# zouyunkai/MedicalSemSeg

Measured on AMD Instinct MI355X. Metric: 96^3 vols/sec fwd+bwd (train), higher is better.
Workload: dtype bf16; 1 GPU; UNet base (MONAI BasicUNet 32-32-64-128-256-32) 1->3cls, 96^3 patches, DiceCE + AdamW, per-GPU batch 2; global_batch=2, parallelism=dp1, grad_sync=none (single rank)

## Files before the change

medicalsemseg_amd/csrc/common.h:

```cpp
#pragma once
#include <hip/hip_runtime.h>
#include <stdint.h>
#include <stdio.h>

#include "../../include/msseg.h"

typedef __bf16 bf16_t;
typedef __attribute__((ext_vector_type(8))) __bf16 bf16x8_t;
typedef __attribute__((ext_vector_type(4))) __bf16 bf16x4_t;
typedef __attribute__((ext_vector_type(4))) float f32x4_t;
typedef __attribute__((ext_vector_type(4))) uint32_t u32x4_t;
typedef __attribute__((ext_vector_type(2))) uint32_t u32x2_t;

#define MSSEG_DEVFN __device__ __forceinline__

void msseg_set_error(const char* fmt, ...);
#define MSSEG_FAIL(code, ...)           \
    do {                                \
        msseg_set_error(__VA_ARGS__);   \
        return (code);                  \
    } while (0)
#define MSSEG_CHECK_LAUNCH(name)                                              \
    do {                                                                      \
        hipError_t e__ = hipGetLastError();                                   \
        if (e__ != hipSuccess) MSSEG_FAIL(MSSEG_ELAUNCH, "%s: %s", name, hipGetErrorString(e__)); \
    } while (0)

bool msseg_ktimer_on();
int msseg_ktimer_begin(const char* name, hipStream_t stream);
void msseg_ktimer_end(int slot, hipStream_t stream);
#define MSSEG_KTIMED(name, stream, launch_stmt)                               \
    do {                                                                      \
        const int kt__ = msseg_ktimer_on() ? msseg_ktimer_begin(name, stream) : -1; \
        launch_stmt;                                                          \
        if (kt__ >= 0) msseg_ktimer_end(kt__, stream);                        \
    } while (0)

#include <atomic>
struct msseg_lds_attr_once {
    std::atomic<unsigned long long> done{0};
    bool ensure(const void* kern, int bytes) {
        int dev = 0;
        if (hipGetDevice(&dev) != hipSuccess) return false;
        const bool tracked = dev >= 0 && dev < 64;
        if (tracked && ((done.load(std::memory_order_acquire) >> dev) & 1ull)) return true;
        if (hipFuncSetAttribute(kern, hipFuncAttributeMaxDynamicSharedMemorySize, bytes) != hipSuccess) return false;
        if (tracked) done.fetch_or(1ull << dev, std::memory_order_release);
        return true;
    }
};

template <typename T> struct DT;
template <> struct DT<float> {
    static constexpr int EPC = 4;
    static constexpr int CODE = MSSEG_F32;
    static MSSEG_DEVFN float ld(const float* p) { return *p; }
    static MSSEG_DEVFN void st(float* p, float v) { *p = v; }
};
template <> struct DT<bf16_t> {
    static constexpr int EPC = 8;
    static constexpr int CODE = MSSEG_BF16;
    static MSSEG_DEVFN float ld(const bf16_t* p) { return (float)*p; }
    static MSSEG_DEVFN void st(bf16_t* p, float v) { *p = (bf16_t)v; }
};

template <typename T> MSSEG_DEVFN void mma_chunk(f32x4_t& acc, const u32x4_t& a, const u32x4_t& b);
template <> MSSEG_DEVFN void mma_chunk<bf16_t>(f32x4_t& acc, const u32x4_t& a, const u32x4_t& b) {
    acc = __builtin_amdgcn_mfma_f32_16x16x32_bf16(__builtin_bit_cast(bf16x8_t, a), __builtin_bit_cast(bf16x8_t, b),
                                                  acc, 0, 0, 0);
}
template <> MSSEG_DEVFN void mma_chunk<float>(f32x4_t& acc, const u32x4_t& a, const u32x4_t& b) {
    f32x4_t af = __builtin_bit_cast(f32x4_t, a), bf = __builtin_bit_cast(f32x4_t, b);
#pragma unroll
    for (int j = 0; j < 4; ++j) acc = __builtin_amdgcn_mfma_f32_16x16x4f32(af[j], bf[j], acc, 0, 0, 0);
}

MSSEG_DEVFN u32x4_t ldg16(const void* p) { return *(const u32x4_t*)p; }

MSSEG_DEVFN long long wimg_frag_off(int blk, int nkb, int kb, int q, int cb, int row) {
    return ((((long long)blk * nkb + kb) * 4 + q) * cb + row) * 16;
}
MSSEG_DEVFN long long wimg_kblock_bytes(int cb) { return (long long)4 * cb * 16; }

MSSEG_DEVFN bf16x4_t lds_tr_read(const unsigned char* p) {
    return __builtin_amdgcn_ds_read_tr16_b64_v4bf16(
        (__attribute__((address_space(3))) bf16x4_t*)(uintptr_t)(uint32_t)(uintptr_t)p);
}
MSSEG_DEVFN u32x4_t tr_frag(const unsigned char* base, int r0, int r1) {
    const bf16x4_t lo = lds_tr_read(base + r0), hi = lds_tr_read(base + r1);
    const bf16x8_t f = {lo[0], lo[1], lo[2], lo[3], hi[0], hi[1], hi[2], hi[3]};
    return __builtin_bit_cast(u32x4_t, f);
}

static inline bool msseg_aligned_bf16(int dtype, const void* a, long long lda, int ca, const void* b, long long ldb, int cb) {
    return dtype == MSSEG_BF16 && !((lda % 8) || (ldb % 8) || ((uintptr_t)a & 15) || ((uintptr_t)b & 15) || lda < ca || ldb < cb);
}

template <typename T> struct Chunk;
template <> struct Chunk<bf16_t> {
    static constexpr int E = 8;
    static MSSEG_DEVFN void load(const bf16_t* p, float* f) {
        const bf16x8_t v = *(const bf16x8_t*)p;
#pragma unroll
        for (int e = 0; e < 8; ++e) f[e] = (float)v[e];
    }
    static MSSEG_DEVFN void store(bf16_t* p, const float* f) {
        bf16x8_t v;
#pragma unroll
        for (int e = 0; e < 8; ++e) v[e] = (bf16_t)f[e];
        *(bf16x8_t*)p = v;
    }
};
template <> struct Chunk<float> {
    static constexpr int E = 4;
    static MSSEG_DEVFN void load(const float* p, float* f) {
        const f32x4_t v = *(const f32x4_t*)p;
#pragma unroll
        for (int e = 0; e < 4; ++e) f[e] = v[e];
    }
    static MSSEG_DEVFN void store(float* p, const float* f) { *(f32x4_t*)p = f32x4_t{f[0], f[1], f[2], f[3]}; }
};

template <typename T> MSSEG_DEVFN void load4(const T* p, float* f);
template <> MSSEG_DEVFN void load4<float>(const float* p, float* f) { Chunk<float>::load(p, f); }
template <> MSSEG_DEVFN void load4<bf16_t>(const bf16_t* p, float* f) {
    const bf16x4_t v = *(const bf16x4_t*)p;
#pragma unroll
    for (int e = 0; e < 4; ++e) f[e] = (float)v[e];
}
template <typename T> MSSEG_DEVFN void store4(T* p, const float* f);
template <> MSSEG_DEVFN void store4<float>(float* p, const float* f) { Chunk<float>::store(p, f); }
template <> MSSEG_DEVFN void store4<bf16_t>(bf16_t* p, const float* f) {
    *(bf16x4_t*)p = bf16x4_t{(bf16_t)f[0], (bf16_t)f[1], (bf16_t)f[2], (bf16_t)f[3]};
}

MSSEG_DEVFN float wave_sum(float v) {
#pragma unroll
    for (int o = 32; o > 0; o >>= 1) v += __shfl_xor(v, o);
    return v;
}

MSSEG_DEVFN bool grid_last_block(unsigned int* counter, unsigned int total_blocks, int* lds_flag) {
    asm volatile("s_waitcnt vmcnt(0)" ::: "memory");
    __syncthreads();
    if (threadIdx.x == 0) {
        __builtin_amdgcn_fence(__ATOMIC_RELEASE, "agent");
        asm volatile("s_waitcnt vmcnt(0)" ::: "memory");
        const unsigned int prev = __hip_atomic_fetch_add(counter, 1u, __ATOMIC_RELAXED, __HIP_MEMORY_SCOPE_AGENT);
        const int last = (prev == total_blocks - 1u) ? 1 : 0;
        if (last) {
            __builtin_amdgcn_fence(__ATOMIC_ACQUIRE, "agent");
            asm volatile("s_waitcnt vmcnt(0)" ::: "memory");
            __hip_atomic_store(counter, 0u, __ATOMIC_RELAXED, __HIP_MEMORY_SCOPE_AGENT);
        }
        *lds_flag = last;
    }
    __syncthreads();
    return *lds_flag != 0;
}

template <int NT>
MSSEG_DEVFN void block_rows_sum(const float* rows, int R, int L, float* lds, long long stride = 0) {
    const int tid = threadIdx.x, q = L >> 2;
    const int SL = NT / q;
    const int c4 = tid % q, slot = tid / q;
    const long long q_stride = (stride ? stride : (long long)L) >> 2;
    f32x4_t* l4 = (f32x4_t*)lds;
    if (slot < SL) {
        f32x4_t acc = {0.f, 0.f, 0.f, 0.f};
        const f32x4_t* src = (const f32x4_t*)rows + c4;
#pragma unroll 8
        for (int x = slot; x < R; x += SL) acc += src[(long long)x * q_stride];
        l4[slot * q + c4] = acc;
    }
    __syncthreads();
    if (tid < q) {
        f32x4_t t = {0.f, 0.f, 0.f, 0.f};
        for (int sl = 0; sl < SL; ++sl) t += l4[sl * q + tid];
        l4[NT + tid] = t;
    }
    __syncthreads();
}

#define MSSEG_SCRATCH_COUNTER_BYTES 256
#define MSSEG_STATS_NMAX 8

static inline int scratch_ok(const void* scratch, size_t bytes, const char* who) {
    if (!scratch || ((uintptr_t)scratch & 255) || bytes < msseg_reduce_scratch_bytes())
        MSSEG_FAIL(MSSEG_EWORKSPACE, "%s: needs a zero-initialised, 256-byte aligned scratch of %zu bytes", who,
                   msseg_reduce_scratch_bytes());
    return MSSEG_OK;
}

static inline int ceil_div(int a, int b) { return (a + b - 1) / b; }
static inline long long ceil_div_ll(long long a, long long b) { return (a + b - 1) / b; }

static inline int stream_grid(long long items, long long items_per_block = 256) {
    long long b = ceil_div_ll(items, items_per_block);
    const long long cap = (long long)msseg_num_cus() * 16;
    if (b > cap) b = cap;
    return (int)(b < 1 ? 1 : b);
}

static inline int epc_of(int dtype) { return dtype == MSSEG_F32 ? 4 : 8; }

template <typename T> struct type_tag { using type = T; };
template <typename F> static inline bool for_dtype(int dtype, F&& f) {
    if (dtype == MSSEG_F32) f(type_tag<float>{});
    else if (dtype == MSSEG_BF16) f(type_tag<bf16_t>{});
    else return false;
    return true;
}
```

medicalsemseg_amd/csrc/elementwise.hip:

```cpp
#include "common.h"

#include <stdarg.h>
#include <string.h>

static thread_local char g_err[512] = "";
void msseg_set_error(const char* fmt, ...) {
    va_list ap;
    va_start(ap, fmt);
    vsnprintf(g_err, sizeof(g_err), fmt, ap);
    va_end(ap);
}

extern "C" {
int msseg_abi_version(void) { return MSSEG_ABI_VERSION; }
const char* msseg_last_error(void) { return g_err; }
int msseg_num_cus(void) {
    static int cus = 0;
    if (cus == 0) {
        int dev = 0;
        hipDeviceProp_t prop;
        if (hipGetDevice(&dev) == hipSuccess && hipGetDeviceProperties(&prop, dev) == hipSuccess)
            cus = prop.multiProcessorCount;
        if (cus <= 0) cus = 256;
    }
    return cus;
}
}

namespace {

template <typename T> struct ChunkV {
    static constexpr int EPC = DT<T>::EPC;
    float v[EPC];
    MSSEG_DEVFN void load(const T* p) { Chunk<T>::load(p, v); }
    MSSEG_DEVFN void store(T* p) const { Chunk<T>::store(p, v); }
};

inline bool vec_ok(const void* p, long long ld, int C, int esz) {
    const int epc = 16 / esz;
    return (C % epc) == 0 && (ld % epc) == 0 && (((uintptr_t)p) & 15) == 0;
}

struct RowMap {
    int groups;
    int rows_par;
};
inline RowMap row_map(int C, int width, int nthr = 256) {
    RowMap m;
    m.groups = ceil_div(C, width);
    if (m.groups > nthr) m.groups = nthr;
    m.rows_par = nthr / m.groups;
    if (m.rows_par < 1) m.rows_par = 1;
    return m;
}

MSSEG_DEVFN void finalize_channels(const float* ws, int N, int nblk, int C, int nper, int mode, float* out,
                                   float* dp0, float* dp1, int accumulate) {
    __shared__ float fin[256];
    const int L = C * nper;
    const int cols = L < 256 ? L : 256;
    const int G = 256 / cols;
    const int col = threadIdx.x % cols, rg = threadIdx.x / cols;
    const bool in256 = threadIdx.x < 256;
    const int n_step = mode == 0 ? (int)gridDim.y : 1, n_first = mode == 0 ? (int)blockIdx.y : 0;
    for (int c0 = blockIdx.x * cols; c0 < L; c0 += gridDim.x * cols) {
        const int o = c0 + col;
        const bool ok = in256 && o < L && rg < G;
        float tot = 0.f;
        for (int n = n_first; n < N; n += n_step) {
            float s = 0.f;
            if (ok) {
                const float* src = ws + (long long)n * nblk * L + o;
#pragma unroll 16
                for (int bb = rg; bb < nblk; bb += G) s += src[(long long)bb * L];
            }
            __syncthreads();
            if (in256) fin[threadIdx.x] = s;
            __syncthreads();
            if (ok && rg == 0) {
                float t = 0.f;
                for (int g = 0; g < G; ++g) t += fin[g * cols + col];
                if (mode != 1) out[(long long)n * L + o] = t;
                tot += t;
            }
        }
        if (ok && rg == 0) {
            if (mode == 1) {
                out[o] = accumulate ? out[o] + tot : tot;
            } else if (mode == 2) {
                const int c = o / nper, k = o % nper;
                float* dp = (k == 0) ? dp0 : dp1;
                if (dp) dp[c] = accumulate ? dp[c] + tot : tot;
            }
        }
    }
}

struct FinalizeArgs {
    const float* ws; int N, nblk, C, nper, mode; float* out; float* dp0; float* dp1; int accumulate;
};
__global__ __launch_bounds__(256) void channels_finalize_kernel(const FinalizeArgs a) {
    finalize_channels(a.ws, a.N, a.nblk, a.C, a.nper, a.mode, a.out, a.dp0, a.dp1, a.accumulate);
}

static inline dim3 channels_finalize_grid(const FinalizeArgs& a) {
    const int L = a.C * a.nper;
    int gx = (L + 255) / 256;
    if (gx > 64) gx = 64;
    if (gx < 1) gx = 1;
    return dim3((unsigned)gx, a.mode == 0 ? (unsigned)(a.N < 1 ? 1 : a.N) : 1u);
}

constexpr int RED_THREADS = 512;
constexpr int RED_STAGE2 = 16;

template <int W>
MSSEG_DEVFN void block_rows_reduce(float* red, int groups, int rows_par, int g, int rl, bool act) {
    if (act && rl < RED_STAGE2 && rl < rows_par) {
#pragma unroll
        for (int e = 0; e < W; ++e) {
            float a = 0.f, b = 0.f;
            for (int k = rl; k < rows_par; k += RED_STAGE2) {
                a += red[((k * groups + g) * W + e) * 2 + 0];
                b += red[((k * groups + g) * W + e) * 2 + 1];
            }
            red[((rl * groups + g) * W + e) * 2 + 0] = a;
            red[((rl * groups + g) * W + e) * 2 + 1] = b;
        }
    }
    __syncthreads();
}

template <typename T, bool VEC>
__global__ __launch_bounds__(RED_THREADS) void channel_stats_kernel(const T* __restrict__ x, long long ldx, float* out,
                                                            long long S, int C, int groups, int rows_par,
                                                            long long rows_per_block, int nacc, int accumulate,
                                                            float* ws, unsigned int* counter) {
    constexpr int W = VEC ? DT<T>::EPC : 1;
    __shared__ float red[RED_THREADS * 2 * (VEC ? DT<T>::EPC : 1)];
    __shared__ int lflag;
    const int n = blockIdx.y;
    const int g = threadIdx.x % groups, rl = threadIdx.x / groups;
    const long long r0 = (long long)blockIdx.x * rows_per_block;
    long long r1 = r0 + rows_per_block;
    if (r1 > S) r1 = S;
    const T* xn = x + (long long)n * S * ldx;
    float* wsb = ws + ((long long)n * gridDim.x + blockIdx.x) * C * nacc;
    for (int gbase = 0; gbase * W < C; gbase += groups) {
        const int gg = gbase + g;
        const bool act = gg * W < C;
        float s[W], s2[W];
#pragma unroll
        for (int e = 0; e < W; ++e) s[e] = s2[e] = 0.f;
        if (act && rl < rows_par) {
#pragma unroll 8
            for (long long r = r0 + rl; r < r1; r += rows_par) {
// ... 179 lines not shown
    var = var > 0.f ? var : 0.f;
    rstd = rsqrtf(var + eps);
}

template <typename T, bool VEC, int MODE>
__global__ __launch_bounds__(MODE == 1 ? RED_THREADS : 256) void instnorm_kernel(const NormParams p) {
    constexpr int W = VEC ? DT<T>::EPC : 1;
    __shared__ float red[(MODE == 1) ? RED_THREADS * 2 * W : 1];
    __shared__ int lflag;
    const int n = blockIdx.y;
    const int g = threadIdx.x % p.groups, rl = threadIdx.x / p.groups;
    const long long r0 = (long long)blockIdx.x * p.rows_per_block;
    long long r1 = r0 + p.rows_per_block;
    if (r1 > p.S) r1 = p.S;
    const T* xn = (const T*)p.x + (long long)n * p.S * p.ldx;
    const T* yn = (MODE != 0 && p.y != nullptr) ? (const T*)p.y + (long long)n * p.S * p.ldy : nullptr;
    T* yo = (MODE == 0) ? (T*)p.y + (long long)n * p.S * p.ldy : nullptr;
    const T* dyn = (MODE != 0) ? (const T*)p.dy + (long long)n * p.S * p.lddy : nullptr;
    const T* resn = (MODE == 0 && p.res) ? (const T*)p.res + (long long)n * p.S * p.ldr : nullptr;
    T* dxn = (MODE == 2) ? (T*)p.dx + (long long)n * p.S * p.lddx : nullptr;
    T* drn = (MODE == 2 && p.dres) ? (T*)p.dres + (long long)n * p.S * p.lddres : nullptr;
    const float invS = 1.0f / (float)p.S;

    for (int gbase = 0; gbase * W < p.C; gbase += p.groups) {
        const int gg = gbase + g;
        const bool act = gg * W < p.C;
        float mean[W], rstd[W], sc[W], sh[W], k0[W], k1[W], a0[W], a1[W];
#pragma unroll
        for (int e = 0; e < W; ++e) {
            const int c = act ? gg * W + e : 0;
            mean_rstd(p.stats, n, p.C, c, p.S, p.eps, mean[e], rstd[e]);
            const float ga = p.gamma ? p.gamma[c] : 1.f;
            sc[e] = rstd[e] * ga;
            sh[e] = (p.beta ? p.beta[c] : 0.f) - mean[e] * sc[e];
            a0[e] = a1[e] = 0.f;
            if constexpr (MODE == 2) {
                k0[e] = p.red[((long long)n * p.C + c) * 2 + 0] * invS;
                k1[e] = p.red[((long long)n * p.C + c) * 2 + 1] * invS;
            }
        }
        if (act && rl < p.rows_par) {
#pragma unroll 4
            for (long long r = r0 + rl; r < r1; r += p.rows_par) {
                float xv[W], o[W], yv[W], dv[W];
                if constexpr (VEC) {
                    ChunkV<T> c; c.load(xn + r * p.ldx + gg * W);
#pragma unroll
                    for (int e = 0; e < W; ++e) xv[e] = c.v[e];
                } else {
                    xv[0] = DT<T>::ld(xn + r * p.ldx + gg);
                }
                if constexpr (MODE == 0) {
                    float rv[W];
#pragma unroll
                    for (int e = 0; e < W; ++e) rv[e] = 0.f;
                    if (resn) {
                        if constexpr (VEC) {
                            ChunkV<T> c; c.load(resn + r * p.ldr + gg * W);
#pragma unroll
                            for (int e = 0; e < W; ++e) rv[e] = c.v[e];
                        } else {
                            rv[0] = DT<T>::ld(resn + r * p.ldr + gg);
                        }
                    }
#pragma unroll
                    for (int e = 0; e < W; ++e) {
                        const float z = xv[e] * sc[e] + sh[e] + rv[e];
                        o[e] = z > 0.f ? z : z * p.slope;
                    }
                    if constexpr (VEC) {
                        ChunkV<T> c;
#pragma unroll
                        for (int e = 0; e < W; ++e) c.v[e] = o[e];
                        c.store(yo + r * p.ldy + gg * W);
                    } else {
                        DT<T>::st(yo + r * p.ldy + gg, o[0]);
                    }
                } else {
                    if constexpr (VEC) {
                        ChunkV<T> d; d.load(dyn + r * p.lddy + gg * W);
#pragma unroll
                        for (int e = 0; e < W; ++e) dv[e] = d.v[e];
                        if (yn != nullptr) {
                            ChunkV<T> c; c.load(yn + r * p.ldy + gg * W);
#pragma unroll
                            for (int e = 0; e < W; ++e) yv[e] = c.v[e];
                        } else {
#pragma unroll
                            for (int e = 0; e < W; ++e) yv[e] = xv[e] * sc[e] + sh[e];
                        }
                    } else {
                        dv[0] = DT<T>::ld(dyn + r * p.lddy + gg);
                        yv[0] = (yn != nullptr) ? DT<T>::ld(yn + r * p.ldy + gg) : xv[0] * sc[0] + sh[0];
                    }
#pragma unroll
                    for (int e = 0; e < W; ++e) {
                        const float dz = yv[e] > 0.f ? dv[e] : dv[e] * p.slope;
                        const float xh = (xv[e] - mean[e]) * rstd[e];
                        if constexpr (MODE == 1) {
                            a0[e] += dz;
                            a1[e] += dz * xh;
                        } else {
                            o[e] = sc[e] * (dz - k0[e] - xh * k1[e]);
                            dv[e] = dz;
                        }
                    }
                    if constexpr (MODE == 2) {
                        if constexpr (VEC) {
                            ChunkV<T> c;
#pragma unroll
                            for (int e = 0; e < W; ++e) c.v[e] = o[e];
                            c.store(dxn + r * p.lddx + gg * W);
                            if (drn) {
#pragma unroll
                                for (int e = 0; e < W; ++e) c.v[e] = dv[e];
                                c.store(drn + r * p.lddres + gg * W);
                            }
                        } else {
                            DT<T>::st(dxn + r * p.lddx + gg, o[0]);
                            if (drn) DT<T>::st(drn + r * p.lddres + gg, dv[0]);
                        }
                    }
                }
            }
        }
        if constexpr (MODE == 1) {
            __syncthreads();
#pragma unroll
            for (int e = 0; e < W; ++e) {
                red[(threadIdx.x * W + e) * 2 + 0] = a0[e];
                red[(threadIdx.x * W + e) * 2 + 1] = a1[e];
            }
            __syncthreads();
            block_rows_reduce<W>(red, p.groups, p.rows_par, g, rl, act);
            if (act && rl == 0) {
                const int kmax = p.rows_par < RED_STAGE2 ? p.rows_par : RED_STAGE2;
#pragma unroll
                for (int e = 0; e < W; ++e) {
                    float a = 0.f, b = 0.f;
                    for (int k = 0; k < kmax; ++k) {
                        a += red[((k * p.groups + g) * W + e) * 2 + 0];
                        b += red[((k * p.groups + g) * W + e) * 2 + 1];
                    }
                    const int c = gg * W + e;
                    float* wsb = p.ws + ((long long)n * gridDim.x + blockIdx.x) * p.C * 2;
                    wsb[c * 2 + 0] = a;
                    wsb[c * 2 + 1] = b;
                }
            }
        }
    }
}

struct NormPoolParams {
    const void* x; long long ldx;
    const float* stats; const float* gamma; const float* beta;
    void* y; long long ldy;
    void* pooled; long long ldp;
    int N, D, H, W, C; float eps, slope;
};

template <typename T>
__global__ __launch_bounds__(256) void instnorm_pool_fwd_kernel(const NormPoolParams p) {
    constexpr int WD = DT<T>::EPC;
    const int OD = p.D / 2, OH = p.H / 2, OW = p.W / 2;
    const unsigned ug = (unsigned)(p.C / WD);
    const unsigned total = (unsigned)((long long)p.N * OD * OH * OW * ug);
    const long long S = (long long)p.D * p.H * p.W;
    for (unsigned i = blockIdx.x * 256u + threadIdx.x; i < total; i += gridDim.x * 256u) {
        unsigned t = i / ug;
        const int g = (int)(i - t * ug);
        unsigned t2 = t / (unsigned)OW;
        const int ow = (int)(t - t2 * (unsigned)OW);
        t = t2 / (unsigned)OH;
        const int oh = (int)(t2 - t * (unsigned)OH);
        const int n = (int)(t / (unsigned)OD);
        const int od = (int)(t - (unsigned)n * (unsigned)OD);
        float sc[WD], sh[WD], best[WD];
#pragma unroll
        for (int e = 0; e < WD; ++e) {
            const int c = g * WD + e;
            float mean, rstd;
            mean_rstd(p.stats, n, p.C, c, S, p.eps, mean, rstd);
            sc[e] = rstd * (p.gamma ? p.gamma[c] : 1.f);
            sh[e] = (p.beta ? p.beta[c] : 0.f) - mean * sc[e];
            best[e] = -INFINITY;
        }
        ChunkV<T> in[8];
#pragma unroll
        for (int k = 0; k < 8; ++k) {
            const long long vox = (((long long)n * p.D + 2 * od + (k >> 2)) * p.H + 2 * oh + ((k >> 1) & 1)) * p.W + 2 * ow + (k & 1);
            in[k].load((const T*)p.x + vox * p.ldx + g * WD);
        }
#pragma unroll
        for (int k = 0; k < 8; ++k) {
            const long long vox = (((long long)n * p.D + 2 * od + (k >> 2)) * p.H + 2 * oh + ((k >> 1) & 1)) * p.W + 2 * ow + (k & 1);
            ChunkV<T> o;
#pragma unroll
            for (int e = 0; e < WD; ++e) {
                const float z = in[k].v[e] * sc[e] + sh[e];
                const float a = (float)(T)(z > 0.f ? z : z * p.slope);
                o.v[e] = a;
                if (a > best[e] || a != a) best[e] = a;
            }
            o.store((T*)p.y + vox * p.ldy + g * WD);
        }
        ChunkV<T> b;
#pragma unroll
        for (int e = 0; e < WD; ++e) b.v[e] = best[e];
        const long long ovox = (((long long)n * OD + od) * OH + oh) * OW + ow;
        b.store((T*)p.pooled + ovox * p.ldp + g * WD);
    }
}

struct NormPoolBwdParams {
    const void* x; long long ldx;
    const float* stats; const float* gamma; const float* beta;
    const void* skip; long long lds;
    const void* g; long long ldg;
    void* da; long long ldda;
    int N, D, H, W, C; float eps, slope;
    int groups, rows_par; long long cells_per_block;
    float* ws;
};

template <typename T>
__global__ __launch_bounds__(RED_THREADS) void instnorm_poolbwd_reduce_kernel(const NormPoolBwdParams p) {
    constexpr int WD = DT<T>::EPC;
    __shared__ float red[RED_THREADS * 2 * WD];
    const int n = blockIdx.y;
    const int g = threadIdx.x % p.groups, rl = threadIdx.x / p.groups;
    const int OD = p.D / 2, OH = p.H / 2, OW = p.W / 2;
    const long long cells = (long long)OD * OH * OW, S = (long long)p.D * p.H * p.W;
    const long long c0 = (long long)blockIdx.x * p.cells_per_block;
    long long c1 = c0 + p.cells_per_block;
    if (c1 > cells) c1 = cells;
    const T* xn = (const T*)p.x + (long long)n * S * p.ldx;
    const T* sn = (const T*)p.skip + (long long)n * S * p.lds;
    const T* gn = (const T*)p.g + (long long)n * cells * p.ldg;
    T* dn = (T*)p.da + (long long)n * S * p.ldda;
    for (int gbase = 0; gbase * WD < p.C; gbase += p.groups) {
        const int gg = gbase + g;
        const bool act = gg * WD < p.C;
        float mean[WD], rstd[WD], sc[WD], sh[WD], a0[WD], a1[WD];
#pragma unroll
        for (int e = 0; e < WD; ++e) {
            const int c = act ? gg * WD + e : 0;
            mean_rstd(p.stats, n, p.C, c, S, p.eps, mean[e], rstd[e]);
            sc[e] = rstd[e] * (p.gamma ? p.gamma[c] : 1.f);
            sh[e] = (p.beta ? p.beta[c] : 0.f) - mean[e] * sc[e];
            a0[e] = a1[e] = 0.f;
        }
        if (act && rl < p.rows_par) {
            for (long long cell = c0 + rl; cell < c1; cell += p.rows_par) {
                const int ow = (int)(cell % OW), oh = (int)((cell / OW) % OH), od = (int)(cell / ((long long)OW * OH));
                ChunkV<T> xin[8], gv;
                ChunkV<T> skin[8];
                long long vox[8];
#pragma unroll
                for (int k = 0; k < 8; ++k) {
                    vox[k] = ((long long)(2 * od + (k >> 2)) * p.H + 2 * oh + ((k >> 1) & 1)) * p.W + 2 * ow + (k & 1);
                    xin[k].load(xn + vox[k] * p.ldx + gg * WD);
                }
#pragma unroll
                for (int k = 0; k < 8; ++k) skin[k].load(sn + vox[k] * p.lds + gg * WD);
                gv.load(gn + cell * p.ldg + gg * WD);
                float best[WD];
                int arg[WD];
#pragma unroll
                for (int e = 0; e < WD; ++e) { best[e] = -INFINITY; arg[e] = 0; }
#pragma unroll
                for (int k = 0; k < 8; ++k) {
#pragma unroll
                    for (int e = 0; e < WD; ++e) {
                        const float z = xin[k].v[e] * sc[e] + sh[e];
                        const float a = (float)(T)(z > 0.f ? z : z * p.slope);
                        if (a > best[e] || a != a) { best[e] = a; arg[e] = k; }
                    }
                }
#pragma unroll
                for (int k = 0; k < 8; ++k) {
                    ChunkV<T> o;
#pragma unroll
                    for (int e = 0; e < WD; ++e) {
                        const float dv = (float)(T)(skin[k].v[e] + (arg[e] == k ? gv.v[e] : 0.f));
                        o.v[e] = dv;
                        const float z = xin[k].v[e] * sc[e] + sh[e];
                        const float dz = z > 0.f ? dv : dv * p.slope;
                        a0[e] += dz;
                        a1[e] += dz * ((xin[k].v[e] - mean[e]) * rstd[e]);
                    }
                    o.store(dn + vox[k] * p.ldda + gg * WD);
                }
            }
        }
        __syncthreads();
#pragma unroll
        for (int e = 0; e < WD; ++e) {
            red[(threadIdx.x * WD + e) * 2 + 0] = a0[e];
            red[(threadIdx.x * WD + e) * 2 + 1] = a1[e];
        }
        __syncthreads();
        block_rows_reduce<WD>(red, p.groups, p.rows_par, g, rl, act);
        if (act && rl == 0) {
            const int kmax = p.rows_par < RED_STAGE2 ? p.rows_par : RED_STAGE2;
#pragma unroll
            for (int e = 0; e < WD; ++e) {
                float a = 0.f, b = 0.f;
                for (int k = 0; k < kmax; ++k) {
                    a += red[((k * p.groups + g) * WD + e) * 2 + 0];
                    b += red[((k * p.groups + g) * WD + e) * 2 + 1];
                }
                float* wsb = p.ws + ((long long)n * gridDim.x + blockIdx.x) * p.C * 2;
                wsb[(gg * WD + e) * 2 + 0] = a;
                wsb[(gg * WD + e) * 2 + 1] = b;
            }
        }
    }
}

struct HeadBwdParams {
    const void* dy; long long lddy;
    const float* w;
    const void* x; long long ldx;
    const float* stats; const float* gamma; const float* beta;
    void* da; long long ldda;
    long long S; int C, Cout; float eps, slope;
    int groups, rows_par; long long rows_per_block;
    float* ws;
    int want_dw;
};

struct HeadFinArgs {
    const float* ws; int N, nblk, C, nper, Cout; float* red; float* dbeta; float* dgamma; float* dw; int acc_norm, acc_dw;
};
__global__ __launch_bounds__(256) void head_finalize_kernel(const HeadFinArgs a) {
    __shared__ __attribute__((aligned(16))) float fin[256 * 4 + 64 * 6];
    __shared__ float tot_n[64 * 6];
    const int L = a.C * a.nper;
    for (int o = threadIdx.x; o < L; o += 256) tot_n[o] = 0.f;
    for (int n = 0; n < a.N; ++n) {
        block_rows_sum<256>(a.ws + (long long)n * a.nblk * L, a.nblk, L, fin);
        const float* t = fin + 256 * 4;
        for (int o = threadIdx.x; o < L; o += 256) {
            const int c = o / a.nper, k = o % a.nper;
            if (k < 2) a.red[((long long)n * a.C + c) * 2 + k] = t[o];
            tot_n[o] += t[o];
        }
        __syncthreads();
    }
    for (int o = threadIdx.x; o < L; o += 256) {
        const int c = o / a.nper, k = o % a.nper;
        const float tot = tot_n[o];
        if (k == 0) { if (a.dbeta) a.dbeta[c] = a.acc_norm ? a.dbeta[c] + tot : tot; }
        else if (k == 1) { if (a.dgamma) a.dgamma[c] = a.acc_norm ? a.dgamma[c] + tot : tot; }
        else if (k - 2 < a.Cout && a.dw) a.dw[(k - 2) * a.C + c] = a.acc_dw ? a.dw[(k - 2) * a.C + c] + tot : tot;
    }
}

template <typename T, bool DW>
__global__ __launch_bounds__(RED_THREADS) void head_dgrad_inbwd_kernel(const HeadBwdParams p) {
    constexpr int WD = DT<T>::EPC;
    __shared__ float red[RED_THREADS * 2 * WD];
    const int n = blockIdx.y;
    const int g = threadIdx.x % p.groups, rl = threadIdx.x / p.groups;
    const long long r0 = (long long)blockIdx.x * p.rows_per_block;
    long long r1 = r0 + p.rows_per_block;
    if (r1 > p.S) r1 = p.S;
    const T* xn = (const T*)p.x + (long long)n * p.S * p.ldx;
    const T* dyn = (const T*)p.dy + (long long)n * p.S * p.lddy;
    T* dan = (T*)p.da + (long long)n * p.S * p.ldda;
    for (int gbase = 0; gbase * WD < p.C; gbase += p.groups) {
        const int gg = gbase + g;
        const bool act = gg * WD < p.C;
        float mean[WD], rstd[WD], sc[WD], sh[WD], a0[WD], a1[WD], wv[4][WD];
        float gw[DW ? 4 : 1][WD];
#pragma unroll
        for (int e = 0; e < WD; ++e) {
            const int c = act ? gg * WD + e : 0;
            mean_rstd(p.stats, n, p.C, c, p.S, p.eps, mean[e], rstd[e]);
            sc[e] = rstd[e] * (p.gamma ? p.gamma[c] : 1.f);
            sh[e] = (p.beta ? p.beta[c] : 0.f) - mean[e] * sc[e];
            a0[e] = a1[e] = 0.f;
#pragma unroll
            for (int k = 0; k < 4; ++k) wv[k][e] = k < p.Cout ? (float)(T)p.w[k * p.C + c] : 0.f;
#pragma unroll
            for (int k = 0; k < (DW ? 4 : 1); ++k) gw[k][e] = 0.f;
        }
        if (act && rl < p.rows_par) {
            constexpr int UNR = DW ? 2 : 4;
#pragma unroll UNR
            for (long long r = r0 + rl; r < r1; r += p.rows_par) {
                ChunkV<T> xc, dc, o;
                xc.load(xn + r * p.ldx + gg * WD);
                dc.load(dyn + r * p.lddy);
#pragma unroll
                for (int e = 0; e < WD; ++e) {
                    float acc = 0.f;
#pragma unroll
                    for (int k = 0; k < 4; ++k) acc += dc.v[k] * wv[k][e];
                    const float da = (float)(T)acc;
                    o.v[e] = da;
                    const float z = xc.v[e] * sc[e] + sh[e];
                    const float dz = z > 0.f ? da : da * p.slope;
                    a0[e] += dz;
                    a1[e] += dz * ((xc.v[e] - mean[e]) * rstd[e]);
                    if constexpr (DW) {
                        const float av = (float)(T)(z > 0.f ? z : z * p.slope);
#pragma unroll
                        for (int k = 0; k < 4; ++k) gw[k][e] += dc.v[k] * av;
                    }
                }
                o.store(dan + r * p.ldda + gg * WD);
            }
        }
        constexpr int NPER = DW ? 6 : 2;
        float* wsb = p.ws + ((long long)n * gridDim.x + blockIdx.x) * p.C * NPER;
#pragma unroll
        for (int round = 0; round < NPER / 2; ++round) {
            __syncthreads();
#pragma unroll
            for (int e = 0; e < WD; ++e) {
                float v0, v1;
                if (round == 0) { v0 = a0[e]; v1 = a1[e]; }
                else { v0 = gw[DW ? 2 * round - 2 : 0][e]; v1 = gw[DW ? 2 * round - 1 : 0][e]; }
                red[(threadIdx.x * WD + e) * 2 + 0] = v0;
                red[(threadIdx.x * WD + e) * 2 + 1] = v1;
            }
            __syncthreads();
            block_rows_reduce<WD>(red, p.groups, p.rows_par, g, rl, act);
            if (act && rl == 0) {
                const int kmax = p.rows_par < RED_STAGE2 ? p.rows_par : RED_STAGE2;
#pragma unroll
                for (int e = 0; e < WD; ++e) {
                    float a = 0.f, b = 0.f;
                    for (int k = 0; k < kmax; ++k) {
                        a += red[((k * p.groups + g) * WD + e) * 2 + 0];
                        b += red[((k * p.groups + g) * WD + e) * 2 + 1];
                    }
                    wsb[(gg * WD + e) * NPER + 2 * round + 0] = a;
                    wsb[(gg * WD + e) * NPER + 2 * round + 1] = b;
                }
            }
        }
    }
}

template <typename T, int MODE> int launch_norm(NormParams& p, int N, bool vec, hipStream_t st) {
    constexpr int NTHR = MODE == 1 ? RED_THREADS : 256;
    const RowMap m = row_map(p.C, vec ? DT<T>::EPC : 1, NTHR);
    p.groups = m.groups; p.rows_par = m.rows_par;
    long long blocks;
    if (MODE == 1) {
        blocks = reduce_blocks(p.S, m.rows_par, N, p.C, 2);
    } else {
        blocks = ceil_div_ll(p.S, (long long)m.rows_par * 4);
        const long long cap = (long long)msseg_num_cus() * 8 / (N > 0 ? N : 1);
        if (blocks > cap) blocks = cap;
        if (blocks < 1) blocks = 1;
    }
    p.rows_per_block = ceil_div_ll(p.S, blocks);
    blocks = ceil_div_ll(p.S, p.rows_per_block);
    dim3 grid((unsigned)blocks, N);
    if (vec) hipLaunchKernelGGL((instnorm_kernel<T, true, MODE>), grid, dim3(NTHR), 0, st, p);
    else hipLaunchKernelGGL((instnorm_kernel<T, false, MODE>), grid, dim3(NTHR), 0, st, p);
    MSSEG_CHECK_LAUNCH("instnorm");
    if (MODE == 1) {
        FinalizeArgs a{p.ws, N, (int)blocks, p.C, 2, 2, p.red, p.dbeta, p.dgamma, p.accumulate};
        hipLaunchKernelGGL(channels_finalize_kernel, channels_finalize_grid(a), dim3(256), 0, st, a);
        MSSEG_CHECK_LAUNCH("channels_finalize");
    }
    return MSSEG_OK;
}

template <typename T, bool VEC, bool BWD>
__global__ __launch_bounds__(256) void maxpool2_kernel(const T* __restrict__ x, long long ldx, const T* __restrict__ dy,
                                                       long long lddy, T* __restrict__ out, long long ldo, int N, int D,
                                                       int H, int W, int C, int accumulate) {
    constexpr int WD = VEC ? DT<T>::EPC : 1;
    const int OD = D / 2, OH = H / 2, OW = W / 2;
    const int groups = (C + WD - 1) / WD;
    const unsigned total = (unsigned)((long long)N * OD * OH * OW * groups);
    for (unsigned i = blockIdx.x * 256u + threadIdx.x; i < total; i += gridDim.x * 256u) {
        const unsigned ug = (unsigned)groups;
        unsigned t = i / ug;
        const int g = (int)(i - t * ug);
        unsigned t2 = t / (unsigned)OW;
        const int ow = (int)(t - t2 * (unsigned)OW);
        t = t2 / (unsigned)OH;
        const int oh = (int)(t2 - t * (unsigned)OH);
        const int n = (int)(t / (unsigned)OD);
        const int od = (int)(t - (unsigned)n * (unsigned)OD);
        float best[WD];
        int arg[WD];
#pragma unroll
        for (int e = 0; e < WD; ++e) { best[e] = -INFINITY; arg[e] = 0; }
#pragma unroll
        for (int k = 0; k < 8; ++k) {
            const long long vox = (((long long)n * D + 2 * od + (k >> 2)) * H + 2 * oh + ((k >> 1) & 1)) * W + 2 * ow + (k & 1);
            float v[WD];
            if constexpr (VEC) {
                ChunkV<T> c; c.load(x + vox * ldx + g * WD);
#pragma unroll
                for (int e = 0; e < WD; ++e) v[e] = c.v[e];
            } else {
                v[0] = DT<T>::ld(x + vox * ldx + g);
            }
#pragma unroll
            for (int e = 0; e < WD; ++e)
                if (v[e] > best[e] || v[e] != v[e]) { best[e] = v[e]; arg[e] = k; }
        }
        const long long ovox = (((long long)n * OD + od) * OH + oh) * OW + ow;
        if constexpr (!BWD) {
            if constexpr (VEC) {
                ChunkV<T> c;
#pragma unroll
                for (int e = 0; e < WD; ++e) c.v[e] = best[e];
                c.store(out + ovox * ldo + g * WD);
            } else {
                DT<T>::st(out + ovox * ldo + g, best[0]);
            }
        } else {
            float gv[WD];
            if constexpr (VEC) {
                ChunkV<T> c; c.load(dy + ovox * lddy + g * WD);
#pragma unroll
                for (int e = 0; e < WD; ++e) gv[e] = c.v[e];
            } else {
                gv[0] = DT<T>::ld(dy + ovox * lddy + g);
            }
#pragma unroll
            for (int k = 0; k < 8; ++k) {
                const long long vox = (((long long)n * D + 2 * od + (k >> 2)) * H + 2 * oh + ((k >> 1) & 1)) * W + 2 * ow + (k & 1);
                T* dst = out + vox * ldo + g * WD;
                if constexpr (VEC) {
                    ChunkV<T> c;
                    if (accumulate) c.load(dst);
                    else {
#pragma unroll
                        for (int e = 0; e < WD; ++e) c.v[e] = 0.f;
                    }
#pragma unroll
                    for (int e = 0; e < WD; ++e) if (arg[e] == k) c.v[e] += gv[e];
                    c.store(dst);
                } else {
                    float base = accumulate ? DT<T>::ld(dst) : 0.f;
                    if (arg[0] == k) base += gv[0];
                    DT<T>::st(dst, base);
                }
            }
        }
    }
}

template <typename TS, typename TD_>
__global__ void ncdhw_to_ndhwc_kernel(const TS* __restrict__ src, TD_* __restrict__ dst, long long ldd, int N, int C,
                                      long long S) {
    const long long total = (long long)N * S * C;
    for (long long i = blockIdx.x * 256LL + threadIdx.x; i < total; i += (long long)gridDim.x * 256) {
        const int c = (int)(i % C);
        const long long s = (i / C) % S;
        const long long n = i / ((long long)C * S);
        DT<TD_>::st(dst + (n * S + s) * ldd + c, DT<TS>::ld(src + (n * C + c) * S + s));
    }
}
template <typename TS, typename TD_>
__global__ void ndhwc_to_ncdhw_kernel(const TS* __restrict__ src, long long lds, TD_* __restrict__ dst, int N, int C,
                                      long long S) {
    const long long total = (long long)N * S * C;
    for (long long i = blockIdx.x * 256LL + threadIdx.x; i < total; i += (long long)gridDim.x * 256) {
        const long long s = i % S;
        const int c = (int)((i / S) % C);
        const long long n = i / ((long long)C * S);
        DT<TD_>::st(dst + (n * C + c) * S + s, DT<TS>::ld(src + (n * S + s) * lds + c));
    }
}

template <typename T>
__global__ void zero_stuff2_kernel(const T* __restrict__ dy, long long lddy, T* __restrict__ out, long long ldo, int N,
                                   int OD, int OH, int OW, int ID, int IH, int IW, int C) {
    const long long total = (long long)N * ID * IH * IW * C;
    for (long long i = blockIdx.x * 256LL + threadIdx.x; i < total; i += (long long)gridDim.x * 256) {
        const int c = (int)(i % C);
        long long t = i / C;
        const int w = (int)(t % IW); t /= IW;
        const int h = (int)(t % IH); t /= IH;
        const int d = (int)(t % ID);
        const int n = (int)(t / ID);
        float v = 0.f;
        if (!(d & 1) && !(h & 1) && !(w & 1) && d / 2 < OD && h / 2 < OH && w / 2 < OW)
            v = DT<T>::ld(dy + ((((long long)n * OD + d / 2) * OH + h / 2) * OW + w / 2) * lddy + c);
        DT<T>::st(out + ((((long long)n * ID + d) * IH + h) * IW + w) * ldo + c, v);
    }
}

template <typename T>
__global__ void add_kernel(const T* a, long long lda, const T* b, long long ldb, T* y, long long ldy, long long rows,
                           int C) {
    const long long total = rows * C;
    for (long long i = blockIdx.x * 256LL + threadIdx.x; i < total; i += (long long)gridDim.x * 256) {
        const int c = (int)(i % C);
        const long long r = i / C;
        DT<T>::st(y + r * ldy + c, DT<T>::ld(a + r * lda + c) + DT<T>::ld(b + r * ldb + c));
    }
}

template <typename T>
__global__ __launch_bounds__(256) void add_vec_kernel(const T* __restrict__ a, long long lda, const T* __restrict__ b,
                                                      long long ldb, T* __restrict__ y, long long ldy, long long rows, int cpr) {
    constexpr int EPC = DT<T>::EPC;
    const long long total = rows * cpr;
    for (long long i = blockIdx.x * 256LL + threadIdx.x; i < total; i += (long long)gridDim.x * 256) {
        const long long r = i / cpr;
        const int c = (int)(i - r * cpr) * EPC;
        ChunkV<T> ca, cb, o;
        ca.load(a + r * lda + c);
        cb.load(b + r * ldb + c);
#pragma unroll
// ... 730 lines not shown
```

Measured before the change: 545.4 vol/s.

## Add batched streaming instance-norm kernel for vectorized forward and backward-apply modes

Adds a dedicated streaming kernel for the instance-norm apply passes (forward normalize+residual+leaky-relu and backward dx computation). Each thread issues four independent 16-byte loads per input stream before doing any math, so several memory requests are in flight per thread. Per-channel scale, shift and backward constants are computed once per channel group. The grid is sized from occupancy (capped at two blocks per CU) and row runs are aligned to the unroll trip. The cost is more template variants and register pressure, and the old vectorized path for these modes is bypassed.

```diff
diff --git a/medicalsemseg_amd/csrc/common.h b/medicalsemseg_amd/csrc/common.h
--- a/medicalsemseg_amd/csrc/common.h
+++ b/medicalsemseg_amd/csrc/common.h
@@ -104,6 +104,11 @@
 #pragma unroll
         for (int e = 0; e < 8; ++e) f[e] = (float)v[e];
     }
+    static MSSEG_DEVFN void unpack(const u32x4_t& raw, float* f) {
+        const bf16x8_t v = __builtin_bit_cast(bf16x8_t, raw);
+#pragma unroll
+        for (int e = 0; e < 8; ++e) f[e] = (float)v[e];
+    }
     static MSSEG_DEVFN void store(bf16_t* p, const float* f) {
         bf16x8_t v;
 #pragma unroll
@@ -115,6 +120,11 @@
     static constexpr int E = 4;
     static MSSEG_DEVFN void load(const float* p, float* f) {
         const f32x4_t v = *(const f32x4_t*)p;
+#pragma unroll
+        for (int e = 0; e < 4; ++e) f[e] = v[e];
+    }
+    static MSSEG_DEVFN void unpack(const u32x4_t& raw, float* f) {
+        const f32x4_t v = __builtin_bit_cast(f32x4_t, raw);
 #pragma unroll
         for (int e = 0; e < 4; ++e) f[e] = v[e];
     }
diff --git a/medicalsemseg_amd/csrc/elementwise.hip b/medicalsemseg_amd/csrc/elementwise.hip
--- a/medicalsemseg_amd/csrc/elementwise.hip
+++ b/medicalsemseg_amd/csrc/elementwise.hip
@@ -2,6 +2,8 @@
 
 #include <stdarg.h>
 #include <string.h>
+
+#include <initializer_list>
 
 static thread_local char g_err[512] = "";
 void msseg_set_error(const char* fmt, ...) {
@@ -487,6 +489,130 @@
     }
 }
 
+constexpr int NORM_U = 4;
+constexpr int NORM_BLOCKS_PER_CU = 2;
+
+template <typename T, int MODE, bool OPT, bool DRES, bool TAIL>
+MSSEG_DEVFN void norm_stream_batch(const char* __restrict__ xb, unsigned ldx, const char* __restrict__ ob, unsigned ldo,
+                                   const char* __restrict__ dyb, unsigned lddy, char* __restrict__ outb, unsigned ldout,
+                                   char* __restrict__ drb, unsigned lddr, int rb, int rows_par, int nrows, unsigned cg,
+                                   const float* mean, const float* rstd, const float* sc, const float* sh,
+                                   const float* k0, const float* k1, float slope) {
+    constexpr int W = DT<T>::EPC, U = NORM_U;
+    constexpr unsigned ES = sizeof(T);
+    unsigned row[U];
+    bool ok[U];
+    u32x4_t xr[U], dr[U], orw[U];
+#pragma unroll
+    for (int u = 0; u < U; ++u) {
+        const int r = rb + u * rows_par;
+        ok[u] = !TAIL || r < nrows;
+        row[u] = (unsigned)(ok[u] ? r : rb);
+    }
+#pragma unroll
+    for (int u = 0; u < U; ++u) xr[u] = ldg16(xb + (row[u] * ldx + cg) * ES);
+    if constexpr (MODE == 2) {
+#pragma unroll
+        for (int u = 0; u < U; ++u) dr[u] = ldg16(dyb + (row[u] * lddy + cg) * ES);
+    }
+    if constexpr (OPT) {
+#pragma unroll
+        for (int u = 0; u < U; ++u) orw[u] = ldg16(ob + (row[u] * ldo + cg) * ES);
+    }
+#pragma unroll
+    for (int u = 0; u < U; ++u) {
+        float xv[W], o[W], dv[W], yv[W];
+        Chunk<T>::unpack(xr[u], xv);
+        if constexpr (MODE == 0) {
+            float rv[W];
+            if constexpr (OPT) {
+                Chunk<T>::unpack(orw[u], rv);
+            } else {
+#pragma unroll
+                for (int e = 0; e < W; ++e) rv[e] = 0.f;
+            }
+#pragma unroll
+            for (int e = 0; e < W; ++e) {
+                const float z = xv[e] * sc[e] + sh[e] + rv[e];
+                o[e] = z > 0.f ? z : z * slope;
+            }
+        } else {
+            Chunk<T>::unpack(dr[u], dv);
+            if constexpr (OPT) {
+                Chunk<T>::unpack(orw[u], yv);
+            } else {
+#pragma unroll
+                for (int e = 0; e < W; ++e) yv[e] = xv[e] * sc[e] + sh[e];
+            }
+#pragma unroll
+            for (int e = 0; e < W; ++e) {
+                const float dz = yv[e] > 0.f ? dv[e] : dv[e] * slope;
+                const float xh = (xv[e] - mean[e]) * rstd[e];
+                o[e] = sc[e] * (dz - k0[e] - xh * k1[e]);
+                dv[e] = dz;
+            }
+        }
+        if (ok[u]) {
+            Chunk<T>::store((T*)(outb + (row[u] * ldout + cg) * ES), o);
+            if constexpr (DRES) Chunk<T>::store((T*)(drb + (row[u] * lddr + cg) * ES), dv);
+        }
+    }
+}
+
+template <typename T, int MODE, bool OPT, bool DRES>
+__global__ __launch_bounds__(256, 4) void instnorm_stream_kernel(const NormParams p) {
+    static_assert(MODE == 0 || MODE == 2, "streaming modes only");
+    constexpr int W = DT<T>::EPC;
+    const int n = blockIdx.y;
+    const int g = threadIdx.x % p.groups, rl = threadIdx.x / p.groups;
+    const long long r0 = (long long)blockIdx.x * p.rows_per_block;
+    const long long r1 = r0 + p.rows_per_block > p.S ? p.S : r0 + p.rows_per_block;
+    const int nrows = (int)(r1 - r0);
+    if (rl >= p.rows_par || rl >= nrows) return;
+    const long long v0 = ((long long)n * p.S + r0) * (long long)sizeof(T);
+    const char* xb = (const char*)p.x + v0 * p.ldx;
+    const char* ob = nullptr;
+    const char* dyb = nullptr;
+    char* outb;
+    char* drb = nullptr;
+    unsigned ldo = 0, lddy = 0, ldout, lddr = 0;
+    if constexpr (MODE == 0) {
+        if constexpr (OPT) { ob = (const char*)p.res + v0 * p.ldr; ldo = (unsigned)p.ldr; }
+        outb = (char*)p.y + v0 * p.ldy; ldout = (unsigned)p.ldy;
+    } else {
+        if constexpr (OPT) { ob = (const char*)p.y + v0 * p.ldy; ldo = (unsigned)p.ldy; }
+        dyb = (const char*)p.dy + v0 * p.lddy; lddy = (unsigned)p.lddy;
+        outb = (char*)p.dx + v0 * p.lddx; ldout = (unsigned)p.lddx;
+        if constexpr (DRES) { drb = (char*)p.dres + v0 * p.lddres; lddr = (unsigned)p.lddres; }
+    }
+    const float invS = 1.0f / (float)p.S;
+    for (int gg = g; gg * W < p.C; gg += p.groups) {
+        float mean[W], rstd[W], sc[W], sh[W], k0[W], k1[W];
+#pragma unroll
+        for (int e = 0; e < W; ++e) {
+            const int c = gg * W + e;
+            mean_rstd(p.stats, n, p.C, c, p.S, p.eps, mean[e], rstd[e]);
+            const float ga = p.gamma ? p.gamma[c] : 1.f;
+            sc[e] = rstd[e] * ga;
+            sh[e] = (p.beta ? p.beta[c] : 0.f) - mean[e] * sc[e];
+            if constexpr (MODE == 2) {
+                k0[e] = p.red[((long long)n * p.C + c) * 2 + 0] * invS;
+                k1[e] = p.red[((long long)n * p.C + c) * 2 + 1] * invS;
+            } else {
+                k0[e] = k1[e] = 0.f;
+            }
+        }
+        const unsigned cg = (unsigned)(gg * W);
+        int rb = rl;
+        for (; rb + (NORM_U - 1) * p.rows_par < nrows; rb += NORM_U * p.rows_par)
+            norm_stream_batch<T, MODE, OPT, DRES, false>(xb, (unsigned)p.ldx, ob, ldo, dyb, lddy, outb, ldout, drb, lddr, rb,
+                                                         p.rows_par, nrows, cg, mean, rstd, sc, sh, k0, k1, p.slope);
+        if (rb < nrows)
+            norm_stream_batch<T, MODE, OPT, DRES, true>(xb, (unsigned)p.ldx, ob, ldo, dyb, lddy, outb, ldout, drb, lddr, rb,
+                                                        p.rows_par, nrows, cg, mean, rstd, sc, sh, k0, k1, p.slope);
+    }
+}
+
 struct NormPoolParams {
     const void* x; long long ldx;
     const float* stats; const float* gamma; const float* beta;
@@ -781,7 +907,46 @@
     }
 }
 
+template <typename T, int MODE, bool OPT, bool DRES> int launch_norm_stream(NormParams& p, int N, hipStream_t st) {
+    static std::atomic<int> resident{0};
+    int per_cu = resident.load(std::memory_order_relaxed);
+    if (per_cu == 0) {
+        if (hipOccupancyMaxActiveBlocksPerMultiprocessor(&per_cu, (const void*)instnorm_stream_kernel<T, MODE, OPT, DRES>,
+                                                         256, 0) != hipSuccess || per_cu < 1)
+            MSSEG_FAIL(MSSEG_ELAUNCH, "instnorm: no occupancy for the streaming kernel");
+        resident.store(per_cu, std::memory_order_relaxed);
+    }
+    if (per_cu > NORM_BLOCKS_PER_CU) per_cu = NORM_BLOCKS_PER_CU;
+    const RowMap m = row_map(p.C, DT<T>::EPC, 256);
+    p.groups = m.groups; p.rows_par = m.rows_par;
+    long long ldmax = p.ldx > 1 ? p.ldx : 1;
+    for (long long ld : {p.ldr, p.ldy, p.lddy, p.lddx, p.lddres}) ldmax = ld > ldmax ? ld : ldmax;
+    long long blocks = ceil_div_ll(p.S, (long long)m.rows_par * NORM_U);
+    const long long cap = (long long)msseg_num_cus() * per_cu / (N > 0 ? N : 1);
+    if (blocks > cap) blocks = cap;
+    long long max_run = ((long long)1 << 30) / (ldmax * (long long)sizeof(T)) - 1;
+    if (max_run < 1) max_run = 1;
+    if (blocks < ceil_div_ll(p.S, max_run)) blocks = ceil_div_ll(p.S, max_run);
+    if (blocks < 1) blocks = 1;
+    p.rows_per_block = ceil_div_ll(p.S, blocks);
+    const long long trip = (long long)m.rows_par * NORM_U;
+    if (ceil_div_ll(p.rows_per_block, trip) * trip <= max_run) p.rows_per_block = ceil_div_ll(p.rows_per_block, trip) * trip;
+    blocks = ceil_div_ll(p.S, p.rows_per_block);
+    hipLaunchKernelGGL((instnorm_stream_kernel<T, MODE, OPT, DRES>), dim3((unsigned)blocks, N), dim3(256), 0, st, p);
+    MSSEG_CHECK_LAUNCH("instnorm");
+    return MSSEG_OK;
+}
+
 template <typename T, int MODE> int launch_norm(NormParams& p, int N, bool vec, hipStream_t st) {
+    if constexpr (MODE != 1) {
+        if (vec) {
+            const bool opt = MODE == 0 ? p.res != nullptr : p.y != nullptr;
+            if constexpr (MODE == 2) {
+                if (p.dres) return opt ? launch_norm_stream<T, 2, true, true>(p, N, st) : launch_norm_stream<T, 2, false, true>(p, N, st);
+            }
+            return opt ? launch_norm_stream<T, MODE, true, false>(p, N, st) : launch_norm_stream<T, MODE, false, false>(p, N, st);
+        }
+    }
     constexpr int NTHR = MODE == 1 ? RED_THREADS : 256;
     const RowMap m = row_map(p.C, vec ? DT<T>::EPC : 1, NTHR);
     p.groups = m.groups; p.rows_par = m.rows_par;
@@ -797,8 +962,12 @@
     p.rows_per_block = ceil_div_ll(p.S, blocks);
     blocks = ceil_div_ll(p.S, p.rows_per_block);
     dim3 grid((unsigned)blocks, N);
-    if (vec) hipLaunchKernelGGL((instnorm_kernel<T, true, MODE>), grid, dim3(NTHR), 0, st, p);
-    else hipLaunchKernelGGL((instnorm_kernel<T, false, MODE>), grid, dim3(NTHR), 0, st, p);
+    if constexpr (MODE == 1) {
+        if (vec) hipLaunchKernelGGL((instnorm_kernel<T, true, 1>), grid, dim3(NTHR), 0, st, p);
+        else hipLaunchKernelGGL((instnorm_kernel<T, false, 1>), grid, dim3(NTHR), 0, st, p);
+    } else {
+        hipLaunchKernelGGL((instnorm_kernel<T, false, MODE>), grid, dim3(NTHR), 0, st, p);
+    }
     MSSEG_CHECK_LAUNCH("instnorm");
     if (MODE == 1) {
         FinalizeArgs a{p.ws, N, (int)blocks, p.C, 2, 2, p.red, p.dbeta, p.dgamma, p.accumulate};
```

Measured after the change: 559.3 vol/s, median of 6. 2.6% higher.
